# google-research/weatherbenchX

Measured on AMD Instinct MI355X. Metric: grid-point·metric evals/s (0.25° 721×1440×37L) at 1/2/4/8 GPUs; % HBM roofline, higher is better.
Workload: dtype f32+f64

## Files before the change

### weatherbenchx_amd/csrc/wbx_ens_impl.hpp

```cpp
#pragma once
#include <cmath>
#include <cstdlib>

#include "wbx_s1.hpp"
#include "wbx_sortnet3_gen.hpp"

namespace wbx {

constexpr int ENS_MIN_WAVES = 1;

constexpr int WBX_ENS_DIAG_LOADONLY = 99;
constexpr int WBX_ENS_DIAG_PAIRWISE_LDS = 98;
constexpr int WBX_ENS_SKIPNA_SORT = 97;

template <typename T>
struct EnsOpGeneric {
  static constexpr int NIN = 2;
  static constexpr int NLANE = WBX_ENS_LANES;
  static constexpr int NACC = WBX_ENS_LANES;
  static constexpr int XR_UNROLL = 1, XK_UNROLL = 1, MIN_WAVES = 1;

  __device__ __forceinline__ static void values(const S1Args& a, const int64_t (&ro)[WBX_MAX_INPUTS], int64_t x,
                                                double (&val)[NLANE]) {
    const int M = a.M;
    const T* pp = reinterpret_cast<const T*>(a.in[0]) + ro[0] + x * a.xstride[0];
    const double td = (double)(reinterpret_cast<const T*>(a.in[1])[ro[1] + x * a.xstride[1]]);
    const bool skip = a.flags & WBX_FLAG_SKIPNA_ENS;
    double se = 0.0, sq = 0.0, sabs = 0.0, pair_total = 0.0, x0 = 0.0;
    int n = 0;
    for (int i = 0; i < M; ++i) {
      const double xi = (double)pp[(int64_t)i * a.mstride];
      if (skip && xi != xi) continue;
      if (n == 0) x0 = xi;
      ++n;
      const double e = xi - x0;
      se += e;
      sq = fma(e, e, sq);
      sabs += fabs(xi - td);
      double row = 0.0;
      for (int j = 0; j < i; ++j) {
        const double xj = (double)pp[(int64_t)j * a.mstride];
        if (skip && xj != xj) continue;
        row += fabs(xi - xj);
      }
      pair_total += row;
    }
    const double dM = (double)n;
    const double fair = (a.flags & WBX_FLAG_FAIR) ? 1.0 : 0.0;
    const double mean_e = se / dM;
    const double mean_d = (x0 - td) + mean_e;
    const double var = (sq - se * mean_e) / (dM - 1.0);
    val[0] = sabs / dM;
    val[1] = 2.0 * pair_total / (dM * (dM - fair));
    val[2] = var;
    val[3] = mean_d * mean_d - var / dM;
    val[4] = mean_d * mean_d;
  }

  template <int V, bool XK>
  __device__ __forceinline__ static void accum(const S1Args& a, const int64_t (&ro)[WBX_MAX_INPUTS], int64_t x,
                                               double (&acc)[XK ? V : 1][NACC]) {
    static_assert(V == 1, "ensemble op is one point per lane");
    double val[NLANE];
    values(a, ro, x, val);
#pragma unroll
    for (int l = 0; l < NLANE; ++l) acc[0][l] += val[l];
  }
};

template <int MP, bool EXACT, int ALGO>
struct EnsOpF32 {
  static constexpr int NIN = 2;
  static constexpr int NLANE = WBX_ENS_LANES;
  static constexpr int NACC = WBX_ENS_LANES;
  static constexpr int XR_UNROLL = 1, XK_UNROLL = 1, MIN_WAVES = ENS_MIN_WAVES;

  struct Regs {
    float xm[MP];
    float t;
    float poison;
  };

  __device__ __forceinline__ static void load(const S1Args& a, const int64_t (&ro)[WBX_MAX_INPUTS], int64_t x, Regs& r) {
    const int M = EXACT ? MP : a.M;
    const float* pp = reinterpret_cast<const float*>(a.in[0]) + ro[0] + x * a.xstride[0];
    r.t = ld_stream(reinterpret_cast<const float*>(a.in[1]) + ro[1] + x * a.xstride[1]);
#pragma unroll
    for (int m = 0; m < MP; ++m) r.xm[m] = (EXACT || m < M) ? ld_stream(pp + (int64_t)m * a.mstride) : INFINITY;
  }

  __device__ __forceinline__ static void values(const S1Args& a, const int64_t (&ro)[WBX_MAX_INPUTS], int64_t x,
                                                double (&val)[NLANE]) {
    Regs r;
    load(a, ro, x, r);
    finish(a, ro, x, r, val);
  }

  template <bool FAST32 = false>
  __device__ __forceinline__ static bool compute(const S1Args& a, Regs& r, double (&val)[NLANE]) {
    const int M = EXACT ? MP : a.M;
    const double td = (double)r.t;
    float(&xm)[MP] = r.xm;

    if constexpr (ALGO == WBX_ENS_DIAG_LOADONLY) {
      float s = 0.f;
#pragma unroll
      for (int m = 0; m < MP; ++m)
        if (EXACT || m < M) s += xm[m];
      val[0] = (double)s - td;
      val[1] = val[2] = val[3] = val[4] = 0.0;
      return false;
    }
    double pair_total = 0.0;
    float poison = 0.f;
    int nvalid = 0;
    bool weird = false;
    float shift32 = 0.f;
    if constexpr (ALGO == WBX_ENS_SKIPNA_SORT) {
      const bool tfin32 = (r.t - r.t) == 0.f;
      shift32 = r.t;
      if (__builtin_amdgcn_ballot_w64(!tfin32)) {
        float lo = INFINITY;
#pragma unroll
        for (int m = 0; m < MP; ++m)
          if (EXACT || m < M) lo = fminf(lo, xm[m]);
        shift32 = tfin32 ? r.t : lo;
      }
#pragma unroll
      for (int m = 0; m < MP; ++m) {
        if (EXACT || m < M) {
          const float x = xm[m];
          const bool missing = x != x;
          nvalid += missing ? 0 : 1;
          xm[m] = missing ? shift32 : x;
        }
      }
      if constexpr (!EXACT) {
        float big = 0.f;
        int m = 0;
        for (; m + 1 < MP; m += 2) {
          const float a = m < M ? xm[m] : 0.f, b = m + 1 < M ? xm[m + 1] : 0.f;
          asm("v_max3_f32 %0, %1, |%2|, |%3|" : "=v"(big) : "v"(big), "v"(a), "v"(b));
        }
        if (m < MP) {
          const float a = m < M ? xm[m] : 0.f;
          asm("v_max3_f32 %0, %1, |%2|, |%2|" : "=v"(big) : "v"(big), "v"(a));
        }
        weird = big == INFINITY;
      }
    }
    if constexpr (ALGO == WBX_ENS_PAIRWISE) {
#pragma unroll
      for (int i = 1; i < MP; ++i) {
        if (EXACT || i < M) {
          float row = 0.f;
#pragma unroll
          for (int j = 0; j < i; ++j) row += fabsf(xm[i] - xm[j]);
          pair_total += (double)row;
        }
      }
    } else if constexpr (ALGO == WBX_ENS_SORT || ALGO == WBX_ENS_SKIPNA_SORT) {
      if constexpr (ALGO == WBX_ENS_SORT) {
        typedef float pk2 __attribute__((ext_vector_type(2)));
        pk2 pz = {0.f, 0.f};
#pragma unroll
        for (int m = 0; m + 1 < MP; m += 2) {
          const pk2 x2 = {xm[m], (EXACT || m + 1 < M) ? xm[m + 1] : 0.f};
          if (EXACT || m < M) pz = x2 * (pk2){0.f, 0.f} + pz;
        }
        if ((MP & 1) && (EXACT || MP - 1 < M)) pz.x = fmaf(xm[MP - 1], 0.f, pz.x);
        poison = pz.x + pz.y;
      }
      auto mn = [](float u, float v) {
        float r;
        asm("v_min_f32 %0, %1, %2" : "=v"(r) : "v"(u), "v"(v));
        return r;
      };
      auto mx = [](float u, float v) {
        float r;
        asm("v_max_f32 %0, %1, %2" : "=v"(r) : "v"(u), "v"(v));
        return r;
      };
      SortNet3<MP>::sort(
          xm, mn, mx,
          [](float u, float v, float w) {
            float r;
            asm("v_min3_f32 %0, %1, %2, %3" : "=v"(r) : "v"(u), "v"(v), "v"(w));
            return r;
          },
          [](float u, float v, float w) {
            float r;
            asm("v_med3_f32 %0, %1, %2, %3" : "=v"(r) : "v"(u), "v"(v), "v"(w));
            return r;
          },
          [](float u, float v, float w) {
            float r;
            asm("v_max3_f32 %0, %1, %2, %3" : "=v"(r) : "v"(u), "v"(v), "v"(w));
            return r;
          });
    }

    bool redo = false;
    if constexpr (ALGO == WBX_ENS_SKIPNA_SORT) {
      if constexpr (EXACT) weird = xm[0] == -INFINITY || xm[MP - 1] == INFINITY;
      stats_skipna(a, xm, nvalid, td, shift32, val);
      r.poison = 0.f;
      return weird;
    }
    if constexpr (FAST32 && EXACT && ALGO == WBX_ENS_SORT) {
      const float range = xm[MP - 1] - xm[0];
      const float big = fmaxf(fmaxf(fabsf(xm[0]), fabsf(xm[MP - 1])), fabsf(r.t));
      const bool fast_ok = (range == 0.f || (range >= 0x1p-50f && range <= 0x1p60f)) && big <= 0x1p100f;
      redo = __builtin_amdgcn_ballot_w64(!fast_ok) != 0;
      if (!redo) stats32(a, xm, r.t, poison, val);
      r.poison = poison;
    } else {
      stats64(a, xm, td, pair_total, val);
      r.poison = poison;
      apply_poison(r, val);
    }
    return redo;
  }

  __device__ __forceinline__ static void apply_poison(const Regs& r, double (&val)[NLANE]) {
    if constexpr (ALGO == WBX_ENS_SORT) {
      if (r.poison != r.poison) {
#pragma unroll
        for (int l = 0; l < NLANE; ++l) val[l] = (double)r.poison;
      }
    }
  }

  template <bool FAST32 = false>
  __device__ __forceinline__ static void finish(const S1Args& a, const int64_t (&ro)[WBX_MAX_INPUTS], int64_t x, Regs& r,
                                                double (&val)[NLANE]) {
    if (compute<FAST32>(a, r, val)) {
      EnsOpGeneric<float>::values(a, ro, x, val);
      apply_poison(r, val);
    }
  }

  __device__ __forceinline__ static double recip_small(double n) {
    double r = __builtin_amdgcn_rcp(n);
    r = fma(fma(-n, r, 1.0), r, r);
    r = fma(fma(-n, r, 1.0), r, r);
    return r;
  }
  __device__ __forceinline__ static void stats_skipna(const S1Args& a, const float (&xm)[MP], const int n, const double td,
                                                      const float shift32, double (&val)[NLANE]) {
    const int M = EXACT ? MP : a.M;
    const double shift = (double)shift32;
    const double x0t = shift - td;
    const double dM = (double)n, dK = (double)(M - n);
    double se = 0.0, sq = 0.0, sabs = 0.0, dot1 = 0.0;
#pragma unroll
    for (int m = 0; m < MP; ++m) {
      if (EXACT || m < M) {
        const double e = (double)xm[m] - shift;
        se += e;
        sq = fma(e, e, sq);
        sabs += fabs(e);
        dot1 = fma((double)(2 * m + 1), e, dot1);
      }
    }
    const double dot = fma(-dM, se, fma(-dK, sabs + se, dot1));
    sabs += n > 0 ? fabs(x0t) : 0.0;
    const double nan = __builtin_nan("");
    const double inv_n = n > 0 ? recip_small(dM) : nan;
    const double inv_n1 = n > 1 ? recip_small(dM - 1.0) : nan;
    const double inv_pairs = (a.flags & WBX_FLAG_FAIR) ? inv_n * inv_n1 : inv_n * inv_n;
    const double mean_e = se * inv_n;
    const double mean_d = x0t + mean_e;
    const double var = (sq - se * mean_e) * inv_n1;
    val[0] = sabs * inv_n;
    val[1] = 2.0 * dot * inv_pairs;
    val[2] = var;
    val[3] = mean_d * mean_d - var * inv_n;
    val[4] = mean_d * mean_d;
  }

  __device__ __forceinline__ static void stats64(const S1Args& a, float (&xm)[MP], const double td, const double pair_total,
                                                 double (&val)[NLANE]) {
    const int M = EXACT ? MP : a.M;
    const double x0 = (double)xm[0];
    const bool tfin = (td - td) == 0.0;
    const double shift = tfin ? td : x0;
    const double x0t = shift - td;
    double se = 0.0, sq = 0.0, sabs = 0.0, dot = 0.0;
#pragma unroll
    for (int m = 0; m < MP; ++m) {
      if (EXACT || m < M) {
        const double e = (double)xm[m] - shift;
        se += e;
        sq = fma(e, e, sq);
        sabs += fabs(e);
        if constexpr (ALGO == WBX_ENS_SORT) dot = fma((double)(2 * (m + 1) - M - 1), e, dot);
      }
    }
    sabs += fabs(x0t);
    const double dM = (double)M;
    const double fair = (a.flags & WBX_FLAG_FAIR) ? 1.0 : 0.0;
    const double inv_m = 1.0 / dM, inv_m1 = M > 1 ? 1.0 / (dM - 1.0) : __builtin_nan(""), spread_scale = 2.0 / (dM * (dM - fair));
    const double mean_e = se * inv_m;
    const double mean_d = x0t + mean_e;
    const double var = (sq - se * mean_e) * inv_m1;
    double spread;
    if constexpr (ALGO == WBX_ENS_SORT) {
      spread = dot * spread_scale;
    } else {
      spread = pair_total * spread_scale;
    }
    if constexpr (ALGO == WBX_ENS_DIAG_PAIRWISE_LDS) {
      static_assert(EXACT && MP % 17 == 0, "the LDS-tiled diagnostic is instantiated for M = 51");
      constexpr int B = 17, NB = MP / B;
      __shared__ float tile[MP][64];
      float* col = &tile[0][threadIdx.x];
#pragma unroll
      for (int m = 0; m < MP; ++m) col[m * 64] = xm[m];
      asm volatile("" ::: "memory");
      double total = 0.0;
#pragma unroll
      for (int bi = 0; bi < NB; ++bi) {
        float xi[B];
#pragma unroll
        for (int k = 0; k < B; ++k) xi[k] = col[(bi * B + k) * 64];
#pragma unroll
        for (int k = 1; k < B; ++k) {
          float row = 0.f;
#pragma unroll
          for (int l = 0; l < k; ++l) row += fabsf(xi[k] - xi[l]);
          total += (double)row;
        }
#pragma unroll
        for (int bj = 0; bj < bi; ++bj) {
          float xj[B];
#pragma unroll
          for (int l = 0; l < B; ++l) xj[l] = col[(bj * B + l) * 64];
#pragma unroll
          for (int k = 0; k < B; ++k) {
            float row = 0.f;
#pragma unroll
            for (int l = 0; l < B; ++l) row += fabsf(xi[k] - xj[l]);
            total += (double)row;
          }
        }
      }
      spread = total * spread_scale;
    }
    val[0] = sabs * inv_m;
    val[1] = spread;
    val[2] = var;
    val[3] = mean_d * mean_d - var * inv_m;
    val[4] = mean_d * mean_d;
  }

  __device__ __forceinline__ static void stats32(const S1Args& a, float (&xm)[MP], const float t, const float poison,
                                                 double (&val)[NLANE]) {
    static_assert(EXACT, "fp32 chain sums are instantiated for the exact-M buckets");
    constexpr int K = 8, MID = MP / 2, NPAIR = MP / 2;
    const float c = xm[MID];
    float se[K], sq[K], sa[K], dt[K];
#pragma unroll
    for (int k = 0; k < K; ++k) se[k] = sq[k] = sa[k] = dt[k] = k == 0 ? poison : 0.f;
#pragma unroll
    for (int i = 0; i < NPAIR; ++i) {
      const int j = MP - 1 - i, k = i % K;
      const float ei = xm[i] - c, ej = xm[j] - c;
      se[k] += ei + ej;
      sq[k] = fmaf(ei, ei, sq[k]);
      sq[k] = fmaf(ej, ej, sq[k]);
      sa[k] += fabsf(xm[i] - t);
      sa[k] += fabsf(xm[j] - t);
      dt[k] = fmaf((float)(MP - 1 - 2 * i), xm[j] - xm[i], dt[k]);
    }
    if constexpr (MP & 1) {
      sa[NPAIR % K] += fabsf(c - t);
    } else {
    }
    auto fold = [](const float (&v)[K]) {
      return ((double)(v[0] + v[4]) + (double)(v[1] + v[5])) + ((double)(v[2] + v[6]) + (double)(v[3] + v[7]));
    };
    const double dse = fold(se), dsq = fold(sq), dsa = fold(sa), ddt = fold(dt);
    constexpr double dM = (double)MP;
    const double fair = (a.flags & WBX_FLAG_FAIR) ? 1.0 : 0.0;
    constexpr double inv_m = 1.0 / dM, inv_m1 = 1.0 / (dM - 1.0);
    const double spread_scale = 2.0 / (dM * (dM - fair));
    const double mean_e = dse * inv_m;
    const double mean_d = ((double)c - (double)t) + mean_e;
    const double var = (dsq - dse * mean_e) * inv_m1;
    val[0] = dsa * inv_m;
    val[1] = ddt * spread_scale;
    val[2] = var;
    val[3] = mean_d * mean_d - var * inv_m;
    val[4] = mean_d * mean_d;
  }

  template <int V, bool XK>
  __device__ __forceinline__ static void accum(const S1Args& a, const int64_t (&ro)[WBX_MAX_INPUTS], int64_t x,
                                               double (&acc)[XK ? V : 1][NACC]) {
    static_assert(V == 1, "ensemble op is one point per lane");
    double val[NLANE];
    values(a, ro, x, val);
#pragma unroll
    for (int l = 0; l < NLANE; ++l) acc[0][l] += val[l];
  }
};

template <class Core, bool SKIPNA>
struct EnsMasked {
  static constexpr int NIN = Core::NIN;
  static constexpr int NLANE = Core::NLANE;
  static constexpr int NACC = Core::NLANE + (SKIPNA ? Core::NLANE : 1);
  static constexpr int XR_UNROLL = 1, XK_UNROLL = 1, MIN_WAVES = ENS_MIN_WAVES;

  __device__ __forceinline__ static void values(const S1Args& a, const int64_t (&ro)[WBX_MAX_INPUTS], int64_t x,
                                                double (&val)[NLANE]) {
    Core::values(a, ro, x, val);
  }

  template <int V, bool XK>
  __device__ __forceinline__ static void accum(const S1Args& a, const int64_t (&ro)[WBX_MAX_INPUTS], int64_t x,
                                               double (&acc)[XK ? V : 1][NACC]) {
    static_assert(V == 1, "ensemble op is one point per lane");
    double val[NLANE];
    Core::values(a, ro, x, val);
    const bool valid =
        (a.flags & WBX_FLAG_MASKED) ? reinterpret_cast<const uint8_t*>(a.in[3])[ro[3] + x * a.xstride[3]] != 0 : true;
    if constexpr (!SKIPNA) {
#pragma unroll
      for (int l = 0; l < NLANE; ++l) acc[0][l] += valid ? val[l] : 0.0;
      acc[0][NLANE] += valid ? 1.0 : 0.0;
    } else {
#pragma unroll
      for (int l = 0; l < NLANE; ++l) {
        const bool ok = valid && !(val[l] != val[l]);
        acc[0][l] += ok ? val[l] : 0.0;
        acc[0][NLANE + l] += ok ? 1.0 : 0.0;
      }
    }
  }
};


#pragma clang diagnostic push
#pragma clang diagnostic ignored "-Winline-asm"
constexpr int ENS_PIPE_NLDS = 50;
constexpr int ENS_PIPE_WAVES = 3;
constexpr int ENS_PIPE_SKIPNA_WAVES = 3;
template <int MP, bool EXACT, int ALGO, bool FLAT>
__global__ void __launch_bounds__(64, ALGO == WBX_ENS_SKIPNA_SORT ? ENS_PIPE_SKIPNA_WAVES : ENS_PIPE_WAVES)
ens_pipe_kernel(S1Args a, int R) {
  using Op = EnsOpF32<MP, EXACT, ALGO>;
  constexpr int NA = Op::NACC;
  constexpr int NLDS = MP < ENS_PIPE_NLDS ? MP : ENS_PIPE_NLDS;
  constexpr int NREG = MP - NLDS;
  __shared__ float stage[NLDS][64];
  const int lane = threadIdx.x;
  const int M = EXACT ? MP : a.M;
  const int64_t b = blockIdx.x;
  const int64_t key = b / a.nchunk;
  const int chunk = (int)(b - key * a.nchunk);
  const int64_t d0 = (int64_t)chunk * a.dchunk;
  const int64_t d1 = d0 + a.dchunk < a.D ? d0 + a.dchunk : a.D;
  const int nx = (int)a.nx;
  const uint32_t lds0 = (uint32_t)(uintptr_t)(__attribute__((address_space(3))) void*)&stage[0][0];
  const int64_t mstride_b = a.mstride * 4;

  int64_t kb[WBX_MAX_INPUTS], ro[WBX_MAX_INPUTS];
  key_bases<2>(a, key, kb);
  double acc[NA];
#pragma unroll
  for (int l = 0; l < NA; ++l) acc[l] = 0.0;

  int64_t d = d0, e0 = 0, e1 = 0, et = 0;
  int wm = 0;
  const int wstep = 64 % nx;
  auto open_segment = [&]() {
    if constexpr (FLAT) {
      const int64_t plane = d / R;
      const int64_t j0 = d - plane * R;
      const int64_t nj = d1 - d < R - j0 ? d1 - d : R - j0;
      row_bases<2>(a, kb, key, plane * R, ro);
      e0 = j0 * nx;
      e1 = (j0 + nj) * nx;
      et = e0 & ~(int64_t)63;
      wm = (int)((et + lane) % nx);
      d += nj;
    } else {
      row_bases<2>(a, kb, key, d, ro);
      e0 = 0;
      e1 = nx;
      et = 0;
      d += 1;
    }
  };

  float xn[NREG > 0 ? NREG : 1], tn = 0.f;
  double wn = 0.0;
  auto issue = [&]() {
    int64_t e = et + lane;
    e = e < e0 ? e0 : (e < e1 ? e : e1 - 1);
    const uint32_t voff = (uint32_t)e * (uint32_t)a.xstride[0] * 4u;
    const char* um = uniform_ptr(reinterpret_cast<const char*>(a.in[0]) + ro[0] * 4);
#pragma unroll
    for (int m = 0; m < NLDS; ++m) {
      if (EXACT || m < M)
        asm volatile("s_add_u32 m0, %2, %3\n\tglobal_load_lds_dword %0, %1 nt" ::"v"(voff), "s"(um), "s"(lds0), "i"(m * 256)
                     : "memory", "scc", "m0");
      um += mstride_b;
      asm volatile("" : "+s"(um));
    }
    const float* pr = reinterpret_cast<const float*>(a.in[0]) + ro[0] + e * a.xstride[0];
#pragma unroll
    for (int m = NLDS; m < MP; ++m) xn[m - NLDS] = (EXACT || m < M) ? ld_stream(pr + (int64_t)m * a.mstride) : INFINITY;
    tn = ld_stream(reinterpret_cast<const float*>(a.in[1]) + ro[1] + e * a.xstride[1]);
    if constexpr (FLAT) wn = a.xw[wm];
  };

  bool more = d < d1;
  if (more) {
    open_segment();
    issue();
  }
  while (more) {
    typename Op::Regs r;
    asm volatile("s_waitcnt vmcnt(0)" ::: "memory");
#pragma unroll
    for (int m = 0; m < NLDS; ++m) r.xm[m] = (EXACT || m < M) ? stage[m][lane] : INFINITY;
#pragma unroll
    for (int m = NLDS; m < MP; ++m) r.xm[m] = xn[m - NLDS];
    r.t = tn;
    const double wcur = wn;
    const int64_t ecur = et + lane;
    const bool valid = ecur >= e0 && ecur < e1;
    const int64_t xcur = ecur < e0 ? e0 : (ecur < e1 ? ecur : e1 - 1);
    int64_t rocur[WBX_MAX_INPUTS];
#pragma unroll
    for (int i = 0; i < WBX_MAX_INPUTS; ++i) rocur[i] = ro[i];
    const bool full = et >= e0 && et + 64 <= e1;
    et += 64;
    if (et >= e1) {
      more = d < d1;
      if (more) open_segment();
    } else if constexpr (FLAT) {
      wm += wstep;
      wm = wm >= nx ? wm - nx : wm;
    }
    asm volatile("s_waitcnt lgkmcnt(0)" ::: "memory");
    if (more) issue();
    double val[Op::NLANE];
    Op::template finish<true>(a, rocur, xcur, r, val);
    if constexpr (FLAT) {
      if (full) {
#pragma unroll
        for (int l = 0; l < NA; ++l) acc[l] = fma(val[l], wcur, acc[l]);
      } else {
#pragma unroll
        for (int l = 0; l < NA; ++l) acc[l] = fma(valid ? val[l] : 0.0, wcur, acc[l]);
      }
    } else if (full) {
#pragma unroll
      for (int l = 0; l < NA; ++l) acc[l] += val[l];
    } else {
#pragma unroll
      for (int l = 0; l < NA; ++l) acc[l] += valid ? val[l] : 0.0;
    }
  }
#pragma unroll
  for (int l = 0; l < NA; ++l) {
    const double v = wave_sum(acc[l]);
    if (lane == l) a.out[(key * a.nchunk + chunk) * NA + l] = v;
  }
}

#pragma clang diagnostic pop

inline bool ens_pipe_ok(const wbx_s1_plan* plan, const S1Args& a, bool skipna_ens = false) {
  static const bool off = getenv("WBX_ENS_PIPE") && atoi(getenv("WBX_ENS_PIPE")) == 0;
  static const bool off_skipna = getenv("WBX_ENS_PIPE_SKIPNA") && atoi(getenv("WBX_ENS_PIPE_SKIPNA")) == 0;
  if (off || (skipna_ens && off_skipna)) return false;
  if (plan->x_kept || plan->x_weights != nullptr || plan->block_threads != 64) return false;
  if (plan->flags & (WBX_FLAG_MASKED | WBX_FLAG_SKIPNA | (skipna_ens ? 0u : (unsigned)WBX_FLAG_SKIPNA_ENS))) return false;
  if (plan->nx <= 0 || plan->ndepth <= 0 || plan->nkey <= 0) return false;
  if (a.xstride[0] < 0 || a.xstride[1] < 0) return false;
  return (double)plan->nx * (double)a.xstride[0] * 4.0 < 4294967296.0;
}

inline bool ens_pipe_flat_ok(const wbx_s1_plan* plan, const S1Args& a) {
  static const bool off = getenv("WBX_ENS_PIPE") && atoi(getenv("WBX_ENS_PIPE")) == 0;
  if (off) return false;
  if (plan->x_kept || plan->x_weights == nullptr || plan->block_threads != 64 || plan->plane_rows <= 0) return false;
  if (plan->flags & (WBX_FLAG_MASKED | WBX_FLAG_SKIPNA | WBX_FLAG_SKIPNA_ENS)) return false;
  if (plan->nx <= 0 || plan->nx > WBX_XW_MAX || plan->ndepth <= 0 || plan->nkey <= 0 || plan->ndepth % plan->plane_rows != 0) return false;
  if (a.xstride[0] != 1 || a.xstride[1] != 1) return false;
  return (double)plan->nx * (double)plan->plane_rows * 4.0 < 4294967296.0;
}

template <int MP, bool EXACT, int ALGO, bool FLAT = false>
int launch_ens_pipe(wbx_ctx* ctx, const wbx_s1_plan* plan, S1Args& a) {
  const int64_t grid = plan->nkey * plan->nchunk;
  WBX_REQUIRE(grid < (int64_t)1 << 31, "grid too large (%lld blocks)", (long long)grid);
  hipLaunchKernelGGL((ens_pipe_kernel<MP, EXACT, ALGO, FLAT>), dim3((unsigned)grid), dim3(64), 0, ctx->stream, a,
                     FLAT ? plan->plane_rows : 0);
  WBX_HIP(hipGetLastError());
  return 0;
}

template <class Op>
int launch_ens_op(wbx_ctx* ctx, const wbx_s1_plan* plan, S1Args& a, bool map) {
  if (map) return launch_map<Op>(ctx, plan, a);
  if (plan->x_weights != nullptr) {
    WBX_REQUIRE(!(plan->flags & WBX_FLAG_SKIPNA_ENS), "flat x-weighted mode does not take skipna_ensemble");
    if (plan->flags & WBX_FLAG_SKIPNA) return launch_flat_weighted1<EnsMasked<Op, true>>(ctx, plan, a);
    if (plan->flags & WBX_FLAG_MASKED) return launch_flat_weighted1<EnsMasked<Op, false>>(ctx, plan, a);
    return launch_flat_weighted1<Op>(ctx, plan, a);
  }
  if (plan->flags & WBX_FLAG_SKIPNA) return launch_partial<EnsMasked<Op, true>, 1>(ctx, plan, a);
  if (plan->flags & WBX_FLAG_MASKED) return launch_partial<EnsMasked<Op, false>, 1>(ctx, plan, a);
  return launch_partial<Op, 1>(ctx, plan, a);
}

template <int MP, bool EXACT>
int launch_ens_bucket(wbx_ctx* ctx, const wbx_s1_plan* plan, S1Args& a, int algo, bool map) {
  if (!map && algo == WBX_ENS_SORT && ens_pipe_ok(plan, a)) return launch_ens_pipe<MP, EXACT, WBX_ENS_SORT>(ctx, plan, a);
  if (!map && algo == WBX_ENS_SORT && ens_pipe_flat_ok(plan, a)) return launch_ens_pipe<MP, EXACT, WBX_ENS_SORT, true>(ctx, plan, a);
  if (algo == WBX_ENS_SORT) return launch_ens_op<EnsOpF32<MP, EXACT, WBX_ENS_SORT>>(ctx, plan, a, map);
  if (algo == WBX_ENS_DIAG_LOADONLY) {
    if (!EXACT || map) return fail(WBX_ERR_INVALID, "the load-only diagnostic exists for the exact-M partial kernels only");
    return launch_partial<EnsOpF32<MP, EXACT, WBX_ENS_DIAG_LOADONLY>, 1>(ctx, plan, a);
  }
  if (algo == WBX_ENS_DIAG_PAIRWISE_LDS) {
    if constexpr (EXACT && MP == 51) {
      if (map || plan->x_weights != nullptr || (plan->flags & (WBX_FLAG_MASKED | WBX_FLAG_SKIPNA)) || plan->block_threads != 64)
        return fail(WBX_ERR_INVALID, "the LDS-tiled pair-form diagnostic exists for the plain partial kernels with one-wave blocks only");
      return launch_partial<EnsOpF32<MP, EXACT, WBX_ENS_DIAG_PAIRWISE_LDS>, 1>(ctx, plan, a);
    } else {
      return fail(WBX_ERR_INVALID, "the LDS-tiled pair-form diagnostic exists for M = 51 only");
    }
  }
  if (!map && algo == WBX_ENS_SKIPNA_SORT && ens_pipe_ok(plan, a, true)) return launch_ens_pipe<MP, EXACT, WBX_ENS_SKIPNA_SORT>(ctx, plan, a);
  if (algo == WBX_ENS_SKIPNA_SORT) return launch_ens_op<EnsOpF32<MP, EXACT, WBX_ENS_SKIPNA_SORT>>(ctx, plan, a, map);
  return launch_ens_op<EnsOpF32<MP, EXACT, WBX_ENS_PAIRWISE>>(ctx, plan, a, map);
}

int launch_ens_m4(wbx_ctx*, const wbx_s1_plan*, S1Args&, int, bool);
int launch_ens_m8(wbx_ctx*, const wbx_s1_plan*, S1Args&, int, bool);
int launch_ens_m16(wbx_ctx*, const wbx_s1_plan*, S1Args&, int, bool);
int launch_ens_m32(wbx_ctx*, const wbx_s1_plan*, S1Args&, int, bool);
int launch_ens_m64(wbx_ctx*, const wbx_s1_plan*, S1Args&, int, bool);
int launch_ens_m50(wbx_ctx*, const wbx_s1_plan*, S1Args&, int, bool);
int launch_ens_m51(wbx_ctx*, const wbx_s1_plan*, S1Args&, int, bool);

}
```

Before: 120.6 billion.

## Pair adjacent rows per wave in ensemble pipe kernel when nx%64==32

Adds a paired-row variant of the ensemble pipe kernel. When rows are independent and nx leaves a 32-lane remainder (e.g. 1440), one wave processes two consecutive rows, so the junction tile fills both half-waves instead of idling 32 lanes. Each row's accumulators are flushed separately, and the fast-path redo ballot is evaluated per half-wave at the junction. Blocks near the tail are left unpaired to keep load balance. This adds code complexity and more per-tile index arithmetic.

```diff
diff --git a/weatherbenchx_amd/csrc/wbx_ens_impl.hpp b/weatherbenchx_amd/csrc/wbx_ens_impl.hpp
--- a/weatherbenchx_amd/csrc/wbx_ens_impl.hpp
+++ b/weatherbenchx_amd/csrc/wbx_ens_impl.hpp
@@ -96,8 +96,8 @@
     finish(a, ro, x, r, val);
   }
 
-  template <bool FAST32 = false>
-  __device__ __forceinline__ static bool compute(const S1Args& a, Regs& r, double (&val)[NLANE]) {
+  template <bool FAST32 = false, bool HALVES = false>
+  __device__ __forceinline__ static bool compute(const S1Args& a, Regs& r, double (&val)[NLANE], bool halves = false) {
     const int M = EXACT ? MP : a.M;
     const double td = (double)r.t;
     float(&xm)[MP] = r.xm;
@@ -211,7 +211,13 @@
       const float range = xm[MP - 1] - xm[0];
       const float big = fmaxf(fmaxf(fabsf(xm[0]), fabsf(xm[MP - 1])), fabsf(r.t));
       const bool fast_ok = (range == 0.f || (range >= 0x1p-50f && range <= 0x1p60f)) && big <= 0x1p100f;
-      redo = __builtin_amdgcn_ballot_w64(!fast_ok) != 0;
+      if constexpr (HALVES) {
+        const uint64_t bad = __builtin_amdgcn_ballot_w64(!fast_ok);
+        const uint32_t mine = threadIdx.x < 32 ? (uint32_t)bad : (uint32_t)(bad >> 32);
+        redo = halves ? mine != 0 : bad != 0;
+      } else {
+        redo = __builtin_amdgcn_ballot_w64(!fast_ok) != 0;
+      }
       if (!redo) stats32(a, xm, r.t, poison, val);
       r.poison = poison;
     } else {
@@ -447,7 +453,7 @@
 constexpr int ENS_PIPE_NLDS = 50;
 constexpr int ENS_PIPE_WAVES = 3;
 constexpr int ENS_PIPE_SKIPNA_WAVES = 3;
-template <int MP, bool EXACT, int ALGO, bool FLAT>
+template <int MP, bool EXACT, int ALGO, bool FLAT, bool PAIR = false>
 __global__ void __launch_bounds__(64, ALGO == WBX_ENS_SKIPNA_SORT ? ENS_PIPE_SKIPNA_WAVES : ENS_PIPE_WAVES)
 ens_pipe_kernel(S1Args a, int R) {
   using Op = EnsOpF32<MP, EXACT, ALGO>;
@@ -457,6 +463,118 @@
   __shared__ float stage[NLDS][64];
   const int lane = threadIdx.x;
   const int M = EXACT ? MP : a.M;
+  if constexpr (PAIR) {
+    static_assert(!FLAT && ALGO == WBX_ENS_SORT, "paired rows: the plain rank-form sweep only");
+    const int nx = (int)a.nx;
+    const uint32_t lds0 = (uint32_t)(uintptr_t)(__attribute__((address_space(3))) void*)&stage[0][0];
+    const int64_t mstride_b = a.mstride * 4;
+    const int64_t j = blockIdx.x;
+    const bool has_b = j < R;
+    const int64_t ia = has_b ? 2 * j : j + R;
+    const int64_t ib = has_b ? ia + 1 : ia;
+    int64_t roa[WBX_MAX_INPUTS], rob[WBX_MAX_INPUTS];
+    {
+      int64_t kb[WBX_MAX_INPUTS];
+      const int64_t ka = ia / a.nchunk, kbk = ib / a.nchunk;
+      key_bases<2>(a, ka, kb);
+      row_bases<2>(a, kb, ka, (ia - ka * a.nchunk) * a.dchunk, roa);
+      key_bases<2>(a, kbk, kb);
+      row_bases<2>(a, kb, kbk, (ib - kbk * a.nchunk) * a.dchunk, rob);
+    }
+    const int q = nx >> 6;
+    const int ntile = has_b ? 2 * q + 1 : q + 1;
+    const bool hi = lane >= 32;
+    const int ejn = hi ? (has_b ? lane - 32 : nx - 1) : nx - 32 + lane;
+
+    float xn[NREG > 0 ? NREG : 1], tn = 0.f;
+    auto lds_loads = [&](const int64_t ro0, const uint32_t voff) {
+      const char* um = uniform_ptr(reinterpret_cast<const char*>(a.in[0]) + ro0 * 4);
+#pragma unroll
+      for (int m = 0; m < NLDS; ++m) {
+        if (EXACT || m < M)
+          asm volatile("s_add_u32 m0, %2, %3\n\tglobal_load_lds_dword %0, %1 nt" ::"v"(voff), "s"(um), "s"(lds0), "i"(m * 256)
+                       : "memory", "scc", "m0");
+        um += mstride_b;
+        asm volatile("" : "+s"(um));
+      }
+    };
+    auto issue = [&](const int t) {
+      int64_t e, r0, r1;
+      if (t == q) {
+        e = ejn;
+        r0 = hi ? rob[0] : roa[0];
+        r1 = hi ? rob[1] : roa[1];
+        uint64_t vp = (uint64_t)(reinterpret_cast<const float*>(a.in[0]) + r0 + e * a.xstride[0]);
+#pragma unroll
+        for (int m = 0; m < NLDS; ++m) {
+          if (EXACT || m < M)
+            asm volatile("s_add_u32 m0, %1, %2\n\tglobal_load_lds_dword %0, off nt" ::"v"(vp), "s"(lds0), "i"(m * 256)
+                         : "memory", "scc", "m0");
+          vp += (uint64_t)mstride_b;
+          asm volatile("" : "+v"(vp));
+        }
+      } else {
+        const bool in_a = t < q;
+        e = (in_a ? 64 * t : 64 * (t - q) - 32) + lane;
+        r0 = in_a ? roa[0] : rob[0];
+        r1 = in_a ? roa[1] : rob[1];
+        lds_loads(r0, (uint32_t)e * (uint32_t)a.xstride[0] * 4u);
+      }
+      const float* pr = reinterpret_cast<const float*>(a.in[0]) + r0 + e * a.xstride[0];
+#pragma unroll
+      for (int m = NLDS; m < MP; ++m) xn[m - NLDS] = (EXACT || m < M) ? ld_stream(pr + (int64_t)m * a.mstride) : INFINITY;
+      tn = ld_stream(reinterpret_cast<const float*>(a.in[1]) + r1 + e * a.xstride[1]);
+    };
+    auto flush = [&](const int64_t idx, const double (&acc)[NA]) {
+#pragma unroll
+      for (int l = 0; l < NA; ++l) {
+        const double v = wave_sum(acc[l]);
+        if (lane == l) a.out[idx * NA + l] = v;
+      }
+    };
+
+    double acc[NA];
+#pragma unroll
+    for (int l = 0; l < NA; ++l) acc[l] = 0.0;
+    issue(0);
+    for (int t = 0; t < ntile; ++t) {
+      typename Op::Regs r;
+      asm volatile("s_waitcnt vmcnt(0)" ::: "memory");
+#pragma unroll
+      for (int m = 0; m < NLDS; ++m) r.xm[m] = (EXACT || m < M) ? stage[m][lane] : INFINITY;
+#pragma unroll
+      for (int m = NLDS; m < MP; ++m) r.xm[m] = xn[m - NLDS];
+      r.t = tn;
+      asm volatile("s_waitcnt lgkmcnt(0)" ::: "memory");
+      if (t + 1 < ntile) issue(t + 1);
+      const bool jn = t == q;
+      double val[Op::NLANE];
+      if (Op::template compute<true, true>(a, r, val, jn)) {
+        const bool in_b = jn ? hi : t > q;
+        int64_t rocur[WBX_MAX_INPUTS];
+#pragma unroll
+        for (int i = 0; i < WBX_MAX_INPUTS; ++i) rocur[i] = in_b ? rob[i] : roa[i];
+        const int64_t xcur = jn ? ejn : (t < q ? 64 * t : 64 * (t - q) - 32) + lane;
+        EnsOpGeneric<float>::values(a, rocur, xcur, val);
+        Op::apply_poison(r, val);
+      }
+      if (!jn) {
+#pragma unroll
+        for (int l = 0; l < NA; ++l) acc[l] += val[l];
+      } else {
+#pragma unroll
+        for (int l = 0; l < NA; ++l) acc[l] += hi ? 0.0 : val[l];
+        flush(ia, acc);
+#pragma unroll
+        for (int l = 0; l < NA; ++l) {
+          acc[l] = 0.0;
+          acc[l] += (hi && has_b) ? val[l] : 0.0;
+        }
+      }
+    }
+    if (has_b) flush(ib, acc);
+    return;
+  }
   const int64_t b = blockIdx.x;
   const int64_t key = b / a.nchunk;
   const int chunk = (int)(b - key * a.nchunk);
@@ -600,6 +718,17 @@
 int launch_ens_pipe(wbx_ctx* ctx, const wbx_s1_plan* plan, S1Args& a) {
   const int64_t grid = plan->nkey * plan->nchunk;
   WBX_REQUIRE(grid < (int64_t)1 << 31, "grid too large (%lld blocks)", (long long)grid);
+  if constexpr (!FLAT && ALGO == WBX_ENS_SORT) {
+    const bool one_row = (a.D == 1 && a.nchunk == 1) || (a.dchunk == 1 && a.nchunk == a.D);
+    const int64_t tail = 2 * (int64_t)ctx->num_cus * 4 * ENS_PIPE_WAVES;
+    const int64_t npair = one_row && a.nx % 64 == 32 && grid > tail ? (grid - tail) / 2 : 0;
+    if (npair > 0) {
+      hipLaunchKernelGGL((ens_pipe_kernel<MP, EXACT, ALGO, false, true>), dim3((unsigned)(grid - npair)), dim3(64), 0, ctx->stream,
+                         a, (int)npair);
+      WBX_HIP(hipGetLastError());
+      return 0;
+    }
+  }
   hipLaunchKernelGGL((ens_pipe_kernel<MP, EXACT, ALGO, FLAT>), dim3((unsigned)grid), dim3(64), 0, ctx->stream, a,
                      FLAT ? plan->plane_rows : 0);
   WBX_HIP(hipGetLastError());
```

After: 122.0 billion, median of 6. 1.1% higher.
